# rzninvo/LGU-SLAM

Hardware: AMD Instinct MI355X
Metric: def-corr-sample Mpix·edges/s (48×64 fmap, r=3, L=4) (higher is better)
Workload: dtype f32; 1 GPU; BASELINE config 2: TartanAir-mono shape, 48x64 fmap, L=4, r=3, 20 edges per GPU, fused 4-level deformable sample; edges_per_gpu=20, variant=0, volumes=fmap products + avg_pool pyramid, pyramid_layout=4x8-tiled slices (CorrBlock's own storage; results bit-identical), out_format=planar, library=lgu_corr 0.8.0 gfx950

## Files before the change

### include/lgu_corr.h

```cpp
#ifndef LGU_CORR_H
#define LGU_CORR_H

#ifdef __cplusplus
extern "C" {
#endif

#define LGU_OK 0
#define LGU_E_BADARG 100001
#define LGU_E_UNSUPPORTED 100002

#define LGU_MAX_LEVELS 8
#define LGU_MAX_RADIUS 7

const char* lgu_version(void);
int lgu_debug_knobs_enabled(void);
const char* lgu_error_string(int code);


int lgu_defcorr_fwd_f32(const float* volume, const float* coords, float* offset, float* corr,
                        int E, int H1, int W1, int H2, int W2, int radius, void* stream);

int lgu_defcorr_bwd_f32(const float* volume, const float* coords, float* offset,
                        const float* corr_grad, float* volume_grad, float* offset_grad,
                        int E, int H1, int W1, int H2, int W2, int radius, void* stream);
// ... 59 lines not shown

int lgu_volume_pyramid_f32(const float* means, const float* covs, const float* volume, float* const* levels, int L,
                           int E, int H1, int W1, int H2, int W2, int radius, void* stream);

int lgu_volume_pyramid_tiled_f32(const float* means, const float* covs, const float* volume, float* const* levels,
                                 int L, int E, int H1, int W1, int H2, int W2, int radius, void* stream);

int lgu_volume_pyramid_h16(const float* means, const float* covs, const void* volume, float* const* levels, int L,
                           int E, int H1, int W1, int H2, int W2, int radius, int tiled, void* stream);

int lgu_volume_pyramid_det(const float* means, const float* covs, const void* det, int det_half, const void* volume,
                           int volume_half, float* const* levels, int L, int E, int H1, int W1, int H2, int W2, int radius,
                           int tiled, void* stream);

int lgu_volume_build_pyramid_f32(const float* fmap1, const float* fmap2, const float* means, const float* covs, const void* det,
                                 int det_half, float* const* levels, int L, int E, int C, int H, int W, int radius, void* stream);

int lgu_volume_build_pyramid_h16(const void* feats, void* workspace, const float* means, const float* covs, const void* det,
                                 int det_half, float* const* levels, int L, int E, int C, int H, int W, int radius, void* stream);

int lgu_volume_retile_f32(const float* src, float* dst, long long nslices, int H2, int W2, int to_tiled, void* stream);


int lgu_lowmem_defsample_fwd_f32(const float* fmap1, const float* fmap2, const float* coords,
                                 float* offset, float* corr,
                                 int B, int S, int H1, int W1, int H2, int W2, int C, int NO,
                                 int radius, void* stream);

int lgu_altcorr_fwd_f32(const float* fmap1, const float* fmap2, const float* coords, float* corr,
                        int B, int S, int H1, int W1, int H2, int W2, int C,
                        int radius, void* stream);

int lgu_altcorr_bwd_f32(const float* fmap1, const float* fmap2, const float* coords,
                        const float* corr_grad, float* fmap1_grad, float* fmap2_grad,
                        int B, int S, int H1, int W1, int H2, int W2, int C,
                        int radius, void* stream);

int lgu_lowmem_defsample_fwd_h16(const void* fmap1_half, const void* fmap2_half, const float* coords,
                                 float* offset, float* corr,
                                 int B, int S, int H1, int W1, int H2, int W2, int C, int NO,
                                 int radius, void* stream);
int lgu_altcorr_fwd_h16(const void* fmap1_half, const void* fmap2_half, const float* coords, float* corr,
                        int B, int S, int H1, int W1, int H2, int W2, int C,
                        int radius, void* stream);

int lgu_lowmem_pyramid_fwd_h16(const void* fmap1_half, const void* const* fmap2_half, const float* coords,
                               float* const* offsets, float* out,
                               int L, int lbase, int B, int S, int H1, int W1, const int* H2, const int* W2, int C, int NO,
                               int radius, const long long* ii, const long long* jj, void* stream);
int lgu_lowmem_pyramid_fwd_f32(const float* fmap1, const float* const* fmap2, const float* coords,
                               float* const* offsets, float* out,
                               int L, int lbase, int B, int S, int H1, int W1, const int* H2, const int* W2, int C, int NO,
                               int radius, const long long* ii, const long long* jj, void* stream);

int lgu_lowmem_pyramid_chunked_fwd_h16(const void* fmap1_half, const void* const* fmap2_half, const float* coords,
                                       float* const* offsets, float* out,
                                       int L, int lbase, int B, int S, int H1, int W1, const int* H2, const int* W2, int C, int NO,
                                       int radius, const long long* ii, const long long* jj, void* stream);
int lgu_lowmem_pyramid_chunked_fwd_f32(const float* fmap1, const float* const* fmap2, const float* coords,
                                       float* const* offsets, float* out,
                                       int L, int lbase, int B, int S, int H1, int W1, const int* H2, const int* W2, int C, int NO,
                                       int radius, const long long* ii, const long long* jj, void* stream);

int lgu_lowmem_pyramid_calls_fwd_h16(const void* fmap1_half, const void* const* fmap2_half, const float* coords,
                                     float* const* offsets, float* out,
                                     int L, int lbase, int B, int H1, int W1, const int* H2, const int* W2, int C, int NO,
                                     const int* off_row, int radius, const long long* ii, const long long* jj, int chunked,
                                     void* stream);

int lgu_ba_build_f32(const float* targets, const float* weights, const float* poses, const float* disps,
                     const float* intrinsics, const long long* ii, const long long* jj,
                     float* Hs, float* vs, float* Eii, float* Eij, float* Cii, float* wi, float* scratch,
                     int E, int ht, int wd, void* stream);
int lgu_ba_build_slices(int E);
int lgu_ba_accum_f32(const float* inp, const long long* ptrs, const long long* idxs, float* out, int nout, int D, void* stream);
int lgu_ba_depth_system_f32(const float* Cii, const float* wi, const long long* ptrs, const long long* idxs, const long long* kx,
                            const float* disps, const float* disps_sens, const float* eta, int eta_rows, float* Q, float* w,
                            int K, int HW, void* stream);
int lgu_ba_depth_update_f32(const float* Q, const float* w, const float* dw, const long long* ptrs, const long long* idxs,
                            const long long* kx, float* dz, float* disps, int K, int HW, void* stream);
int lgu_ba_scatter_sum_f64(const float* inp, const long long* ptrs, const long long* idxs, const long long* dst, double* out,
                           int m, int D, double sign, void* stream);
int lgu_ba_eet_f32(const float* E, const float* Q, const long long* idx, float* S, int nblocks, int D, void* stream);
int lgu_ba_ev_f32(const float* E, const float* Q, const float* w, const long long* kk, float* v, int n, int D, void* stream);
int lgu_ba_evt_f32(const float* E, const float* x, const long long* idx, float* dw, int n, int D, int P, void* stream);
int lgu_ba_solve_f64(const double* A, const double* b, float* x, int P, double lm, double ep, void* stream);
long long lgu_ba_solve_blocked_work_doubles(int P);
int lgu_ba_solve_blocked_f64(double* A, const double* b, float* x, double* work, int P, double lm, double ep, void* stream);
int lgu_ba_assemble_f64(const float* Hs, const long long* hptr, const long long* hidx, const float* S, const long long* sptr,
                        const long long* sidx, const float* vs, const long long* vptr, const long long* vidx, const float* sv,
                        const long long* svptr, const long long* svidx, double* Ad, double* b, int P, void* stream);
int lgu_ba_pose_retr_f32(float* poses, const float* dx, int t0, int t1, void* stream);
int lgu_ba_disp_retr_f32(float* disps, const float* dz, const long long* inds, int n, int HW, void* stream);

int lgu_frame_distance_f32(const float* poses, int np, const float* disps, int nd, int ht, int wd, const float* intrinsics,
                           const long long* ii, const long long* jj, int num, float beta, float* dist, void* stream);
int lgu_projmap_f32(const float* poses, int np, const float* disps, int nd, int ht, int wd, const float* intrinsics,
                    const long long* ii, const long long* jj, int num, float* coords, float* valid, void* stream);
int lgu_depth_filter_f32(const float* poses, int np, const float* disps, int nd, int ht, int wd, const float* intrinsics,
                         const long long* ix, const float* thresh, int num, float* counter, void* stream);
int lgu_iproj_f32(const float* poses, int np, const float* disps, int nd, int ht, int wd, const float* intrinsics,
                  float* points, void* stream);

#define LGU_REPROJ_JACOBIAN 1
#define LGU_REPROJ_DEPTH 2
int lgu_projective_transform_f32(const float* poses, const float* disps, const float* intrinsics, const long long* ii,
                                 const long long* jj, int B, int np, int nd, int ni, int ht, int wd, int num, int flags,
                                 float* coords, float* valid, float* Ji, float* Jj, float* Jz, void* stream);
int lgu_motion_features_f32(const float* poses, const float* disps, const float* intrinsics, const long long* ii,
                            const long long* jj, const float* target, int B, int np, int nd, int ni, int ht, int wd, int num,
                            float bound, float* coords1, float* motn, float* valid, void* stream);

#define LGU_UPS_MASK_F16 1
#define LGU_UPS_HALF_WEIGHTS 2
int lgu_scatter_mean_f32(const float* src, const long long* index, int outer, int n, long long inner, int M, float* out,
                         void* stream);
int lgu_scatter_mean_h16(const void* src, const long long* index, int outer, int n, long long inner, int M, void* out,
                         void* stream);
int lgu_cvx_upsample_f32(const float* data, const void* mask, int B, int ht, int wd, int flags, float* out, void* stream);
int lgu_upsample_disps_f32(const float* disps, int N, int ht, int wd, const long long* ix, int U, const void* mask,
                           int flags, float* disps_up, void* stream);

#define LGU_KANGRU_CTX_PIXELS 256
int lgu_kangru_context_f32(const float* net, const float* weight, const float* bias, int E, int HW, float* partial,
                           float* glo, void* stream);
int lgu_kangru_context_h16(const void* net, const void* weight, const void* bias, int E, int HW, float* partial, void* glo,
                           void* stream);
int lgu_kan_heads_f32(const float* glo, const float* grid, const float* wpack, int E, float* out, void* stream);
int lgu_kan_heads_h16(const void* glo, const float* grid, const void* wpack, int E, void* out, void* stream);
int lgu_kangru_gates_f32(const float* cz, const float* cr, const float* kz, const float* kr, const float* net, int E,
                         int HW, float* z, float* net_inp, void* stream);
int lgu_kangru_gates_h16(const void* cz, const void* cr, const void* kz, const void* kr, const void* net, int E, int HW,
                         void* z, void* net_inp, void* stream);
int lgu_kangru_blend_f32(const float* cq, const float* kq, const float* z, const float* net, int E, int HW, float* out,
                         void* stream);
int lgu_kangru_blend_h16(const void* cq, const void* kq, const void* z, const void* net, int E, int HW, void* out,
                         void* stream);

#define LGU_PROXIMITY_SMALL_MAX 4096
long long lgu_proximity_prefix_len(int t, int t0, int rad, int stereo);
long long lgu_proximity_capacity(int t, int t0, int t1, int rad, int stereo, long long max_factors);
long long lgu_proximity_work_bytes(int t, int t0, int t1);
int lgu_proximity_select_small(const float* dist, const long long* known_ii, const long long* known_jj, int num_known, int t,
                               int t0, int t1, int rad, int nms, double thresh, long long max_factors, int stereo,
                               long long* e_ii, long long* e_jj, long long capacity, int* count, void* stream);
int lgu_proximity_keys(const float* dist, const long long* known_ii, const long long* known_jj, int num_known, int t, int t0,
                       int t1, int rad, int nms, double thresh, int stereo, long long* keys, void* work, void* stream);
int lgu_proximity_select_sorted(const long long* sorted_keys, void* work, int t, int t0, int t1, int rad, int nms,
                                long long max_factors, int stereo, long long* e_ii, long long* e_jj, long long capacity,
                                int* count, void* stream);

#define LGU_LIE_SO3 0
#define LGU_LIE_SE3 1
int lgu_lie_inv_f32(int group, const float* G, int n, float* out, void* stream);
int lgu_lie_mul_f32(int group, const float* G, const float* H, int n, float* out, void* stream);
int lgu_lie_retr_f32(int group, const float* G, const float* a, int n, float* out, void* stream);
int lgu_lie_exp_f32(int group, const float* a, int n, float* out, void* stream);
int lgu_lie_log_f32(int group, const float* G, int n, float* out, void* stream);
int lgu_lie_matrix_f32(int group, const float* G, int n, float* out, void* stream);
int lgu_lie_act_f32(int group, const float* G, long long ng, const float* p, int width, long long rows, long long g_div,
                    float* out, void* stream);
int lgu_lie_adj_f32(int group, const float* G, long long ng, const float* a, int transpose, long long rows,
                    long long g_div, float* out, void* stream);

int lgu_instnorm_relu_f32(const float* a, const float* b, float* out, long planes, long hw, float eps, int mode,
                          void* stream);
// ... 98 lines not shown
```

### lgu-slam_amd/_lib.py

```python
import ctypes
import os

from . import _build

_c_float_p = ctypes.POINTER(ctypes.c_float)
_vp = ctypes.c_void_p
_int = ctypes.c_int


class FlowConv7Args(ctypes.Structure):
    _fields_ = [("x", _vp), ("wpack", _vp), ("bias", _vp), ("out", _vp), ("N", _int), ("H", _int), ("W", _int)]


class Conv3Args(ctypes.Structure):
    _fields_ = [("x", _vp), ("wpack", _vp), ("bias", _vp), ("out", _vp), ("N", _int), ("H", _int), ("W", _int),
                ("Cout", _int), ("flags", _int)]


class HeadArgs(ctypes.Structure):
    _fields_ = [("x", _vp), ("wpack", _vp), ("bias", _vp), ("out", _vp), ("N", _int), ("H", _int), ("W", _int),
                ("Cout", _int), ("flags", _int)]


class Conv3FanoutArgs(ctypes.Structure):
    _fields_ = [("x", _vp), ("wpack", _vp * 3), ("bias", _vp * 3), ("out", _vp * 3), ("N", _int), ("H", _int), ("W", _int),
                ("G", _int), ("flags", _int)]


class HeadPairArgs(ctypes.Structure):
    _fields_ = [("x", _vp * 2), ("wpack", _vp * 2), ("bias", _vp * 2), ("out", _vp * 2), ("coords", _vp), ("N", _int), ("H", _int),
                ("W", _int), ("flags", _int)]


class UpmaskArgs(ctypes.Structure):
    _fields_ = [("x", _vp), ("wpack", _vp), ("bias", _vp), ("out", _vp), ("N", _int), ("H", _int), ("W", _int), ("flags", _int)]


class UpmaskUpsArgs(ctypes.Structure):
    _fields_ = [("x", _vp), ("wpack", _vp), ("bias", _vp), ("disps", _vp), ("ix", _vp), ("disps_up", _vp), ("U", _int),
                ("N", _int), ("ht", _int), ("wd", _int), ("flags", _int)]


class Conv1Args(ctypes.Structure):
    _fields_ = [("x", _vp), ("wpack", _vp), ("bias", _vp), ("out", _vp), ("N", _int), ("Cin", _int), ("H", _int), ("W", _int),
                ("flags", _int)]


class GruConvArgs(ctypes.Structure):
    _fields_ = [("seg", _vp * 4), ("wpack", _vp), ("bias", _vp), ("k0", _vp), ("k1", _vp), ("net", _vp), ("z", _vp),
                ("out0", _vp), ("out1", _vp), ("seg_ch", _int * 4), ("nseg", _int), ("N", _int), ("H", _int), ("W", _int),
                ("Cout", _int), ("mode", _int), ("flags", _int)]


SIGNATURES = {
    "lgu_defcorr_fwd_f32": [_vp, _vp, _vp, _vp] + [_int] * 6 + [_vp],
    "lgu_defcorr_bwd_f32": [_vp] * 6 + [_int] * 6 + [_vp],
    "lgu_corridx_fwd_f32": [_vp, _vp, _vp] + [_int] * 6 + [_vp],
    "lgu_corridx_bwd_f32": [_vp] * 4 + [_int] * 6 + [_vp],
    "lgu_gaussmask_fwd_f32": [_vp] * 4 + [_int] * 6 + [_vp],
    "lgu_gaussmask_bwd_f32": [_vp] * 6 + [_int] * 6 + [_vp],
    "lgu_defcorr_pyramid_fwd_f32": [ctypes.POINTER(_vp), _vp, ctypes.POINTER(_vp), _vp, _int, _int, _int, _int,
                                    ctypes.POINTER(_int), ctypes.POINTER(_int), _int, _int, _vp],
    "lgu_defcorr_pyramid_slots_fwd_f32": [ctypes.POINTER(_vp), _vp, _vp, ctypes.POINTER(_vp), _vp, _int, _int, _int, _int,
                                          ctypes.POINTER(_int), ctypes.POINTER(_int), _int, _int, _vp],
    "lgu_volume_pyramid_f32": [_vp, _vp, _vp, ctypes.POINTER(_vp), _int, _int, _int, _int, _int, _int, _int, _vp],
    "lgu_volume_pyramid_tiled_f32": [_vp, _vp, _vp, ctypes.POINTER(_vp), _int, _int, _int, _int, _int, _int, _int, _vp],
    "lgu_volume_pyramid_h16": [_vp, _vp, _vp, ctypes.POINTER(_vp), _int, _int, _int, _int, _int, _int, _int, _int, _vp],
    "lgu_volume_pyramid_det": [_vp, _vp, _vp, _int, _vp, _int, ctypes.POINTER(_vp)] + [_int] * 8 + [_vp],
    "lgu_volume_build_pyramid_f32": [_vp] * 5 + [_int, ctypes.POINTER(_vp)] + [_int] * 6 + [_vp],
    "lgu_volume_build_pyramid_h16": [_vp] * 5 + [_int, ctypes.POINTER(_vp)] + [_int] * 6 + [_vp],
    "lgu_gaussian_params": [_vp] * 5 + [_int] * 4 + [ctypes.c_float, _vp],
    "lgu_probe_mask_scale_f32": [_vp, _vp, _int, _int, _int, _int, _vp],
    "lgu_offset_conv_frames_h16": [_vp] * 7 + [_int] * 5 + [_vp],
    "lgu_offset_heads_mark": [_vp, _vp, _int, _vp, _int, _vp, _vp, _vp],
    "lgu_offset_conv_worklist_h16": [_vp] * 4 + [_int] + [_vp] * 5 + [_int] * 4 + [_vp],
    "lgu_offset_heads_combine_f32": [_vp] * 5 + [_int] * 2 + [_vp, _vp],
    "lgu_offsets_finalize": [_vp] * 5 + [_int] * 7 + [ctypes.c_float, _vp],
    "lgu_offsets_finalize_masked": [_vp] * 3 + [_int] + [_vp] * 3 + [_int] * 7 + [ctypes.c_float, _vp],
    "lgu_volume_retile_f32": [_vp, _vp, ctypes.c_longlong, _int, _int, _int, _vp],
    "lgu_lowmem_defsample_fwd_f32": [_vp] * 5 + [_int] * 9 + [_vp],
    "lgu_altcorr_fwd_f32": [_vp] * 4 + [_int] * 8 + [_vp],
    "lgu_lowmem_defsample_fwd_h16": [_vp] * 5 + [_int] * 9 + [_vp],
    "lgu_altcorr_fwd_h16": [_vp] * 4 + [_int] * 8 + [_vp],
    "lgu_lowmem_pyramid_fwd_h16": [_vp, ctypes.POINTER(_vp), _vp, ctypes.POINTER(_vp), _vp, _int, _int, _int, _int, _int, _int,
                                   ctypes.POINTER(_int), ctypes.POINTER(_int), _int, _int, _int, _vp, _vp, _vp],
    "lgu_lowmem_pyramid_chunked_fwd_h16": [_vp, ctypes.POINTER(_vp), _vp, ctypes.POINTER(_vp), _vp, _int, _int, _int, _int, _int, _int,
                                   ctypes.POINTER(_int), ctypes.POINTER(_int), _int, _int, _int, _vp, _vp, _vp],
    "lgu_lowmem_pyramid_chunked_fwd_f32": [_vp, ctypes.POINTER(_vp), _vp, ctypes.POINTER(_vp), _vp, _int, _int, _int, _int, _int, _int,
                                   ctypes.POINTER(_int), ctypes.POINTER(_int), _int, _int, _int, _vp, _vp, _vp],
    "lgu_lowmem_pyramid_calls_fwd_h16": [_vp, ctypes.POINTER(_vp), _vp, ctypes.POINTER(_vp), _vp, _int, _int, _int, _int, _int,
                                         ctypes.POINTER(_int), ctypes.POINTER(_int), _int, _int, _vp, _int, _vp, _vp, _int, _vp],
    "lgu_lowmem_pyramid_fwd_f32": [_vp, ctypes.POINTER(_vp), _vp, ctypes.POINTER(_vp), _vp, _int, _int, _int, _int, _int, _int,
                                   ctypes.POINTER(_int), ctypes.POINTER(_int), _int, _int, _int, _vp, _vp, _vp],
    "lgu_ba_build_f32": [_vp] * 14 + [_int] * 3 + [_vp],
    "lgu_ba_build_slices": [_int],
    "lgu_ba_accum_f32": [_vp] * 4 + [_int] * 2 + [_vp],
    "lgu_ba_depth_system_f32": [_vp] * 8 + [_int] + [_vp] * 2 + [_int] * 2 + [_vp],
    "lgu_ba_depth_update_f32": [_vp] * 8 + [_int] * 2 + [_vp],
    "lgu_ba_scatter_sum_f64": [_vp] * 5 + [_int] * 2 + [ctypes.c_double, _vp],
    "lgu_ba_eet_f32": [_vp] * 4 + [_int] * 2 + [_vp],
    "lgu_ba_ev_f32": [_vp] * 5 + [_int] * 2 + [_vp],
    "lgu_ba_evt_f32": [_vp] * 4 + [_int] * 3 + [_vp],
    "lgu_ba_solve_f64": [_vp, _vp, _vp, _int, ctypes.c_double, ctypes.c_double, _vp],
    "lgu_ba_solve_blocked_f64": [_vp, _vp, _vp, _vp, _int, ctypes.c_double, ctypes.c_double, _vp],
    "lgu_ba_pose_retr_f32": [_vp] * 2 + [_int] * 2 + [_vp],
    "lgu_ba_assemble_f64": [_vp] * 14 + [_int, _vp],
    "lgu_ba_disp_retr_f32": [_vp] * 3 + [_int] * 2 + [_vp],
    "lgu_altcorr_bwd_f32": [_vp] * 6 + [_int] * 8 + [_vp],
    "lgu_defcorr_pyramid_enc_fwd_f32": [ctypes.POINTER(_vp), _vp, _vp, ctypes.POINTER(_vp), _vp, _vp, _vp, _int, _int, _int,
                                        _int, ctypes.POINTER(_int), ctypes.POINTER(_int), _int, _int, _int, _vp],
    "lgu_frame_distance_f32": [_vp, _int, _vp, _int, _int, _int, _vp, _vp, _vp, _int, ctypes.c_float, _vp, _vp],
    "lgu_projmap_f32": [_vp, _int, _vp, _int, _int, _int, _vp, _vp, _vp, _int, _vp, _vp, _vp],
    "lgu_depth_filter_f32": [_vp, _int, _vp, _int, _int, _int, _vp, _vp, _vp, _int, _vp, _vp],
    "lgu_iproj_f32": [_vp, _int, _vp, _int, _int, _int, _vp, _vp, _vp],
    "lgu_projective_transform_f32": [_vp] * 5 + [_int] * 8 + [_vp] * 6,
    "lgu_motion_features_f32": [_vp] * 6 + [_int] * 7 + [ctypes.c_float] + [_vp] * 4,
    "lgu_scatter_mean_f32": [_vp, _vp, _int, _int, ctypes.c_longlong, _int, _vp, _vp],
    "lgu_scatter_mean_h16": [_vp, _vp, _int, _int, ctypes.c_longlong, _int, _vp, _vp],
    "lgu_cvx_upsample_f32": [_vp, _vp] + [_int] * 4 + [_vp, _vp],
    "lgu_upsample_disps_f32": [_vp, _int, _int, _int, _vp, _int, _vp, _int, _vp, _vp],
    "lgu_kangru_context_f32": [_vp] * 3 + [_int] * 2 + [_vp] * 3,
    "lgu_kangru_context_h16": [_vp] * 3 + [_int] * 2 + [_vp] * 3,
    "lgu_kan_heads_f32": [_vp] * 3 + [_int] + [_vp] * 2,
    "lgu_kan_heads_h16": [_vp] * 3 + [_int] + [_vp] * 2,
    "lgu_kangru_gates_f32": [_vp] * 5 + [_int] * 2 + [_vp] * 3,
    "lgu_kangru_gates_h16": [_vp] * 5 + [_int] * 2 + [_vp] * 3,
    "lgu_kangru_blend_f32": [_vp] * 4 + [_int] * 2 + [_vp] * 2,
    "lgu_kangru_blend_h16": [_vp] * 4 + [_int] * 2 + [_vp] * 2,
    "lgu_proximity_select_small": [_vp] * 3 + [_int] * 6 + [ctypes.c_double, ctypes.c_longlong, _int, _vp, _vp,
                                                            ctypes.c_longlong, _vp, _vp],
    "lgu_proximity_keys": [_vp] * 3 + [_int] * 6 + [ctypes.c_double, _int, _vp, _vp, _vp],
    "lgu_proximity_select_sorted": [_vp] * 2 + [_int] * 5 + [ctypes.c_longlong, _int, _vp, _vp, ctypes.c_longlong, _vp, _vp],
    "lgu_lie_inv_f32": [_int, _vp, _int, _vp, _vp],
    "lgu_lie_mul_f32": [_int, _vp, _vp, _int, _vp, _vp],
    "lgu_lie_retr_f32": [_int, _vp, _vp, _int, _vp, _vp],
    "lgu_lie_exp_f32": [_int, _vp, _int, _vp, _vp],
    "lgu_lie_log_f32": [_int, _vp, _int, _vp, _vp],
    "lgu_lie_matrix_f32": [_int, _vp, _int, _vp, _vp],
    "lgu_lie_act_f32": [_int, _vp, ctypes.c_longlong, _vp, _int, ctypes.c_longlong, ctypes.c_longlong, _vp, _vp],
    "lgu_lie_adj_f32": [_int, _vp, ctypes.c_longlong, _vp, _int, ctypes.c_longlong, ctypes.c_longlong, _vp, _vp],
    "lgu_instnorm_relu_f32": [_vp] * 3 + [ctypes.c_long] * 2 + [ctypes.c_float, _int, _vp],
    "lgu_instnorm_relu_h16": [_vp] * 3 + [ctypes.c_long] * 2 + [ctypes.c_float, _int, _vp],
    "lgu_instnorm_resident_limit": [_int],
    "lgu_image_normalize_u8": [_vp, _vp, ctypes.c_long, ctypes.c_long, _c_float_p, _c_float_p, _vp],
    "lgu_flow_conv7_relu_h16": [FlowConv7Args, _vp],
    "lgu_conv3x3_c128_h16": [Conv3Args, _vp],
    "lgu_head3x3_c128_h16": [HeadArgs, _vp],
    "lgu_conv3x3_fanout_c128_h16": [Conv3FanoutArgs, _vp],
    "lgu_head3x3_pair_c128_h16": [HeadPairArgs, _vp],
    "lgu_gruconv3x3_c448_h16": [GruConvArgs, _vp],
    "lgu_upmask1x1_c128_h16": [UpmaskArgs, _vp],
    "lgu_upmask_upsample_f32": [UpmaskUpsArgs, _vp],
    "lgu_conv1x1_o128_h16": [Conv1Args, _vp],
    "lgu_ba_solve_blocked_work_doubles": [_int],
    "lgu_offsets_finalize_scratch_bytes": [_int],
    "lgu_proximity_prefix_len": [_int] * 4,
    "lgu_proximity_capacity": [_int] * 5 + [ctypes.c_longlong],
    "lgu_proximity_work_bytes": [_int] * 3,
    "lgu_version": [],
    "lgu_error_string": [_int],
    "lgu_debug_knobs_enabled": [],
}
RESTYPES = {name: ctypes.c_longlong for name in (
    "lgu_ba_solve_blocked_work_doubles", "lgu_offsets_finalize_scratch_bytes", "lgu_proximity_prefix_len", "lgu_proximity_capacity",
    "lgu_proximity_work_bytes")}
RESTYPES.update(lgu_instnorm_resident_limit=ctypes.c_long, lgu_version=ctypes.c_char_p, lgu_error_string=ctypes.c_char_p)

_lib = None


class LguLibraryError(RuntimeError):
    pass


class UnsupportedShape(RuntimeError):
    """The kernels do not serve this shape / argument pattern (LGU_E_UNSUPPORTED)."""


LGU_E_BADARG, LGU_E_UNSUPPORTED = 100001, 100002


def so_path():
    return os.environ.get("LGU_LIB_PATH") or _build.SO_PATH
# ... 36 lines not shown
```

### lgu-slam_amd/ba.py

```python
import os

import numpy as np
import torch

from . import _lib
from ._host import CurrentDevice, check_operands
from ._host import ptr as _ptr, stream as _stream

_ALPHA = 0.05


def _segments(ix, jx):
    ix = np.asarray(ix, dtype=np.int64)
    jx = np.asarray(jx, dtype=np.int64)
    order = np.argsort(ix, kind="stable")
    sx = ix[order]
    lo = np.searchsorted(sx, jx, side="left")
    hi = np.searchsorted(sx, jx, side="right")
    cnt = hi - lo
    ptrs = np.concatenate([[0], np.cumsum(cnt)])
    cols = np.concatenate([order[a:b] for a, b in zip(lo, hi)]) if len(jx) and cnt.sum() else np.zeros(0, np.int64)
    return ptrs, cols


class _Accum:

    def __init__(self, lib, ix, jx, dev):
        ptrs, cols = _segments(ix, jx)
        self.lib, self.n = lib, len(jx)
        self.ptrs = torch.from_numpy(np.ascontiguousarray(ptrs, dtype=np.int64)).to(dev)
        self.cols = torch.from_numpy(np.ascontiguousarray(cols if len(cols) else [0], dtype=np.int64)).to(dev)

    def __call__(self, data, st, out=None):
        if out is None:
            out = torch.empty((self.n, data.shape[1]), dtype=torch.float32, device=data.device)
        if self.n:
            _lib.check(self.lib.lgu_ba_accum_f32(_ptr(data), _ptr(self.ptrs), _ptr(self.cols), _ptr(out), self.n, data.shape[1], st),
                       "ba accum")
        return out


class _ScatterSum:

    def __init__(self, lib, dest, dev):
        dest = np.asarray(dest, dtype=np.int64)
        rows = np.nonzero(dest >= 0)[0]
        order = rows[np.argsort(dest[rows], kind="stable")]
        keys, counts = np.unique(dest[order], return_counts=True)
        ptrs = np.concatenate([[0], np.cumsum(counts)]).astype(np.int64)
        self.lib, self.m = lib, len(keys)
        self.ptrs = torch.from_numpy(ptrs).to(dev)
        self.idxs = torch.from_numpy(np.ascontiguousarray(order if len(order) else [0], dtype=np.int64)).to(dev)
        self.dst = torch.from_numpy(np.ascontiguousarray(keys if len(keys) else [0], dtype=np.int64)).to(dev)

    def __call__(self, inp, out, sign, st):
        if self.m:
            D = inp.shape[1]
            _lib.check(self.lib.lgu_ba_scatter_sum_f64(_ptr(inp), _ptr(self.ptrs), _ptr(self.idxs), _ptr(self.dst), _ptr(out), self.m, D,
                                                       float(sign), st), "ba assembly")


def _solve(A, b, lm, ep):
    L = A.clone()
    dg = torch.diagonal(L)
    dg += ep + lm * dg
    chol, info = torch.linalg.cholesky_ex(L)
    if int(info) != 0:
        return torch.zeros_like(b)
    return torch.cholesky_solve(b[:, None], chol)[:, 0]


def _csr(dest, ndst, dev):
    dest = np.asarray(dest, dtype=np.int64)
    rows = np.nonzero((dest >= 0) & (dest < ndst))[0]
    order = rows[np.argsort(dest[rows], kind="stable")]
    ptr = np.concatenate([[0], np.cumsum(np.bincount(dest[order], minlength=ndst))]).astype(np.int64)
    idx = np.ascontiguousarray(order if len(order) else [0], dtype=np.int64)
    return torch.from_numpy(ptr).to(dev), torch.from_numpy(idx).to(dev)


class _Plan:

    def __init__(self, lib, ii_h, jj_h, t0, t1, motion_only, dev):
        P = t1 - t0
        ts_h = np.arange(t0, t1, dtype=np.int64)
        ii_exp_h, jj_exp_h = np.concatenate([ts_h, ii_h]), np.concatenate([ts_h, jj_h])
        kx_h, kk_h = np.unique(ii_exp_h, return_inverse=True)
        kk_h = kk_h.astype(np.int64)
        self.kx = torch.from_numpy(kx_h).to(dev)
        self.kk = torch.from_numpy(kk_h).to(dev)
        self.K = int(kx_h.shape[0])
        bi_h = np.concatenate([ii_h, ii_h, jj_h, jj_h]) - t0
        bj_h = np.concatenate([ii_h, jj_h, ii_h, jj_h]) - t0
        self.csr_H = _csr(np.where((bi_h >= 0) & (bj_h >= 0) & (bi_h < P) & (bj_h < P), bi_h * P + bj_h, -1), P * P, dev)
        self.csr_v = _csr(np.concatenate([ii_h, jj_h]) - t0, P, dev)
        self.csr_S = self.csr_sv = None
        if motion_only:
            return
        ent = np.nonzero((jj_exp_h >= t0) & (jj_exp_h < t1))[0]
        ent = ent[np.argsort(kk_h[ent], kind="stable")]
        _, starts, sizes = np.unique(kk_h[ent], return_index=True, return_counts=True)
        a_l, c_l, k_l = [], [], []
        for s0, m_ in zip(starts, sizes):
            g = ent[s0:s0 + m_]
            ua, uc = np.triu_indices(m_)
            a_l.append(g[ua]); c_l.append(g[uc])
            k_l.append(np.full(len(ua), kk_h[g[0]], np.int64))
        self.have_pairs = len(a_l) > 0
        if self.have_pairs:
            a_n, c_n, k_n = np.concatenate(a_l), np.concatenate(c_l), np.concatenate(k_l)
        else:
            a_n = c_n = k_n = np.zeros(1, np.int64)
        self.trip_t = torch.from_numpy(np.ascontiguousarray(np.stack([a_n, c_n, k_n], 1))).to(dev)
        if self.have_pairs:
            npair = len(a_n)
            d_ac = (jj_exp_h[a_n] - t0) * P + (jj_exp_h[c_n] - t0)
            d_ca = np.where(a_n != c_n, (jj_exp_h[c_n] - t0) * P + (jj_exp_h[a_n] - t0), -1)
            ptr, idx = _csr(np.concatenate([d_ac, d_ca]), P * P, dev)
            self.csr_S = (ptr, torch.where(idx < npair, idx, npair - 1 - idx))
        else:
            self.csr_S = None
        self.csr_sv = _csr(jj_exp_h - t0, P, dev)
        self.jpose = torch.from_numpy(jj_exp_h - t0).to(dev).contiguous()
        self.acc_ii_kx = _Accum(lib, ii_h, kx_h, dev)
        self.acc_ii_ts = _Accum(lib, ii_h, ts_h, dev)
        self.acc_exp_kx = _Accum(lib, ii_exp_h, kx_h, dev)


_PLANS = {}
_PLANS_MAX = 8


def _plan_for(lib, ii, jj, t0, t1, motion_only, dev):
    ii_h, jj_h = ii.cpu().numpy().astype(np.int64), jj.cpu().numpy().astype(np.int64)
    key = (ii_h.tobytes(), jj_h.tobytes(), int(t0), int(t1), bool(motion_only), str(dev))
    plan = _PLANS.pop(key, None)
    if plan is None:
        plan = _Plan(lib, ii_h, jj_h, int(t0), int(t1), bool(motion_only), dev)
        while len(_PLANS) >= _PLANS_MAX:
            _PLANS.pop(next(iter(_PLANS)))
    _PLANS[key] = plan
    return plan


def _run(pl, lib, poses, disps, intrinsics, disps_sens, targets, weights, eta_v, ii, jj, t0, t1, iterations, lm, ep,
         motion_only, hooks=None):
    dev = poses.device
    E = ii.shape[0]
    ht, wd = disps.shape[1:]
    HW = ht * wd
    P = t1 - t0
    f32, f64 = torch.float32, torch.float64
    st = _stream(poses)
    kx, kk = pl.kx, pl.kk
    if not motion_only:
        have_pairs, trip_t, jpose = pl.have_pairs, pl.trip_t, pl.jpose
        acc_ii_kx, acc_ii_ts, acc_exp_kx = pl.acc_ii_kx, pl.acc_ii_ts, pl.acc_exp_kx
        K = pl.K
        Q = torch.empty((K, HW), dtype=f32, device=dev)
        w = torch.empty((K, HW), dtype=f32, device=dev)
    reduce_system, after_depth = hooks if hooks is not None else (None, None)
    Hs = torch.empty((4, max(E, 1), 6, 6), dtype=f32, device=dev)
    vs = torch.empty((2, max(E, 1), 6), dtype=f32, device=dev)
    Eii = torch.empty((max(E, 1), 6, HW), dtype=f32, device=dev)[:E]
    Eall = torch.empty((P + E, 6, HW), dtype=f32, device=dev)
    Eij = Eall[P:]
    scratch = torch.empty((max(E, 1) * lib.lgu_ba_build_slices(E) * 90,), dtype=f32, device=dev)
    Cii = torch.empty((max(E, 1), HW), dtype=f32, device=dev)[:E]
    wi = torch.empty((max(E, 1), HW), dtype=f32, device=dev)[:E]
    dx = torch.zeros((P, 6), dtype=f32, device=dev)
    dz = None
    for _ in range(iterations):
        if E:
          _lib.check(lib.lgu_ba_build_f32(_ptr(targets), _ptr(weights), _ptr(poses), _ptr(disps), _ptr(intrinsics), _ptr(ii),
                                          _ptr(jj), _ptr(Hs), _ptr(vs), _ptr(Eii), _ptr(Eij), _ptr(Cii), _ptr(wi), _ptr(scratch), E, ht, wd,
                                          st),
                     "ba build")
        S = sv = None
        if not motion_only:
            _lib.check(lib.lgu_ba_depth_system_f32(_ptr(Cii), _ptr(wi), _ptr(acc_ii_kx.ptrs), _ptr(acc_ii_kx.cols), _ptr(kx), _ptr(disps),
                                                   _ptr(disps_sens), _ptr(eta_v), eta_v.shape[0], _ptr(Q), _ptr(w), K, HW, st),
                       "ba depth system")
            acc_ii_ts(Eii.view(E, 6 * HW), st, out=Eall[:P].view(P, 6 * HW))
            nE = P + E
            if have_pairs:
                S = torch.empty((trip_t.shape[0], 6, 6), dtype=f32, device=dev)
                _lib.check(lib.lgu_ba_eet_f32(_ptr(Eall), _ptr(Q), _ptr(trip_t), _ptr(S), trip_t.shape[0], HW, st), "ba EEt")
            sv = torch.empty((nE, 6), dtype=f32, device=dev)
            _lib.check(lib.lgu_ba_ev_f32(_ptr(Eall), _ptr(Q), _ptr(w), _ptr(kk), _ptr(sv), nE, HW, st), "ba Ev")
        Ad = torch.empty((6 * P, 6 * P), dtype=f64, device=dev)
        b = torch.empty((P, 6), dtype=f64, device=dev)
        cS, cs = pl.csr_S if S is not None else None, pl.csr_sv if sv is not None else None
        _lib.check(lib.lgu_ba_assemble_f64(_ptr(Hs), _ptr(pl.csr_H[0]), _ptr(pl.csr_H[1]),
                                           _ptr(S) if S is not None else None, _ptr(cS[0]) if cS else None, _ptr(cS[1]) if cS else None,
                                           _ptr(vs), _ptr(pl.csr_v[0]), _ptr(pl.csr_v[1]),
                                           _ptr(sv) if sv is not None else None, _ptr(cs[0]) if cs else None, _ptr(cs[1]) if cs else None,
                                           _ptr(Ad), _ptr(b), P, st), "ba assembly")
        if reduce_system is not None:
            reduce_system(Ad, b)
        dx = torch.empty((P, 6), dtype=f32, device=dev)
        rc = lib.lgu_ba_solve_f64(_ptr(Ad), _ptr(b), _ptr(dx), P, float(lm), float(ep), st)
        if rc == _lib.LGU_E_UNSUPPORTED:
            if os.environ.get("LGU_BA_LIBRARY_SOLVE", "0") != "0":
                dx = _solve(Ad, b.view(-1), lm, ep).view(P, 6).to(f32).contiguous()
            else:
                work = torch.empty(int(lib.lgu_ba_solve_blocked_work_doubles(P)), dtype=f64, device=dev)
                _lib.check(lib.lgu_ba_solve_blocked_f64(_ptr(Ad), _ptr(b), _ptr(dx), _ptr(work), P, float(lm), float(ep), st),
                           "ba blocked solve")
        else:
            _lib.check(rc, "ba solve")
        if not motion_only:
            dw = torch.empty((nE, HW), dtype=f32, device=dev)
            _lib.check(lib.lgu_ba_evt_f32(_ptr(Eall), _ptr(dx), _ptr(jpose), _ptr(dw), nE, HW, P, st), "ba EvT")
            dz = torch.empty((K, HW), dtype=f32, device=dev)
            _lib.check(lib.lgu_ba_depth_update_f32(_ptr(Q), _ptr(w), _ptr(dw), _ptr(acc_exp_kx.ptrs), _ptr(acc_exp_kx.cols), _ptr(kx),
                                                   _ptr(dz), _ptr(disps), K, HW, st), "ba depth update")
            if after_depth is not None:
                after_depth(disps)
        _lib.check(lib.lgu_ba_pose_retr_f32(_ptr(poses), _ptr(dx), t0, t1, st), "ba pose retraction")
    return [dx, dz]


def ba(poses, disps, intrinsics, disps_sens, targets, weights, eta, ii, jj, t0, t1, iterations, lm, ep, motion_only, _hooks=None):
    named = [(poses, "poses"), (disps, "disps"), (intrinsics, "intrinsics"), (disps_sens, "disps_sens")]
    if ii.numel():
        named += [(targets, "targets"), (weights, "weights")]
    check_operands(named)
    check_operands([(ii, "ii")], torch.int64)
    check_operands([(jj, "jj")], torch.int64)
    lib = _lib.load()
    dev = poses.device
    HW = disps.shape[1] * disps.shape[2]
    with CurrentDevice(dev):
        pl = _plan_for(lib, ii, jj, t0, t1, motion_only, dev)
        eta_v = None
        if not motion_only:
            if callable(eta):
                eta = eta(pl.kx)
            eta_v = eta.reshape(-1, HW).to(torch.float32).contiguous()
            if eta_v.shape[0] not in (1, pl.K):
                raise RuntimeError("ba: eta must have one row per depth frame (%d) or one row, got %d" % (pl.K, eta_v.shape[0]))
        return _run(pl, lib, poses, disps, intrinsics, disps_sens, targets, weights, eta_v, ii, jj, t0, t1, iterations, lm, ep,
                    motion_only, _hooks)
```

### lgu-slam_amd/csrc/ba.hip

```cpp
#include "lgu_common.hpp"
#include "se3.hpp"

namespace lgu {

constexpr float BA_MIN_DEPTH = 0.25f;
constexpr int BA_THREADS = 256;

__device__ __forceinline__ void adj_se3(const float* t, const float* q, const float* X, float* Y) {
  const float qinv[4] = {-q[0], -q[1], -q[2], q[3]};
  act_so3(qinv, X, Y);
  act_so3(qinv, X + 3, Y + 3);
  const float u[3] = {t[2] * X[1] - t[1] * X[2], t[0] * X[2] - t[2] * X[0], t[1] * X[0] - t[0] * X[1]};
  float v[3];
  act_so3(qinv, u, v);
  Y[3] += v[0]; Y[4] += v[1]; Y[5] += v[2];
}

template <int N>
__device__ __forceinline__ float block_sums(const float (&v)[N], float* red ) {
  static_assert(N <= BA_THREADS, "one result per thread");
  const int w = threadIdx.x >> 6;
  __syncthreads();
#pragma unroll
  for (int i = 0; i < N; i++) {
// ... 188 lines not shown
    disps[f * D + k] += z;
  }
}

__global__ __launch_bounds__(BA_THREADS) void ba_scatter_sum_kernel(const float* __restrict__ inp, const long long* __restrict__ ptrs,
                                                                    const long long* __restrict__ idxs, const long long* __restrict__ dst,
                                                                    double* __restrict__ out, int m, int D, double sign) {
  const int t = blockIdx.x * BA_THREADS + threadIdx.x;
  if (t >= m * D) return;
  const int j = t / D, k = t - j * D;
  double acc = 0.0;
  for (long long i = ptrs[j]; i < ptrs[j + 1]; i++) acc += (double)inp[(size_t)idxs[i] * D + k];
  out[(size_t)dst[j] * D + k] += sign * acc;
}

__global__ __launch_bounds__(BA_THREADS) void ba_assemble_kernel(const float* __restrict__ Hs, const long long* __restrict__ hptr,
                                                                 const long long* __restrict__ hidx, const float* __restrict__ S,
                                                                 const long long* __restrict__ sptr, const long long* __restrict__ sidx,
                                                                 const float* __restrict__ vs, const long long* __restrict__ vptr,
                                                                 const long long* __restrict__ vidx, const float* __restrict__ sv,
                                                                 const long long* __restrict__ svptr, const long long* __restrict__ svidx,
                                                                 double* __restrict__ Ad, double* __restrict__ b, int P) {
  const long long t = (long long)blockIdx.x * BA_THREADS + threadIdx.x;
  const long long nA = (long long)P * P * 36;
  if (t < nA) {
    const int d = (int)(t / 36), k = (int)(t - (long long)d * 36);
    double a = 0.0;
    for (long long i = hptr[d]; i < hptr[d + 1]; i++) a += (double)Hs[(size_t)hidx[i] * 36 + k];
    double out = 0.0;
    if (hptr[d + 1] > hptr[d]) out += 1.0 * a;
    if (S) {
      double c = 0.0, ct = 0.0;
      bool anyd = false, anyt = false;
      const int kt = (k % 6) * 6 + k / 6;
      for (long long i = sptr[d]; i < sptr[d + 1]; i++) {
        const long long e = sidx[i];
        if (e >= 0) { c += (double)S[(size_t)e * 36 + k]; anyd = true; }
        else { ct += (double)S[(size_t)(-e - 1) * 36 + kt]; anyt = true; }
      }
      if (anyd) out += -1.0 * c;
      if (anyt) out += -1.0 * ct;
    }
    const int bi = d / P, bj = d - bi * P, r = k / 6, cidx = k - r * 6;
    Ad[((size_t)bi * 6 + r) * (6 * P) + bj * 6 + cidx] = out;
  } else if (t < nA + (long long)P * 6) {
    const int u = (int)(t - nA), d = u / 6, k = u - d * 6;
    double a = 0.0;
    for (long long i = vptr[d]; i < vptr[d + 1]; i++) a += (double)vs[(size_t)vidx[i] * 6 + k];
    double out = 0.0;
    if (vptr[d + 1] > vptr[d]) out += 1.0 * a;
    if (sv) {
      double c = 0.0;
      for (long long i = svptr[d]; i < svptr[d + 1]; i++) c += (double)sv[(size_t)svidx[i] * 6 + k];
      if (svptr[d + 1] > svptr[d]) out += -1.0 * c;
    }
    b[u] = out;
  }
}

__global__ __launch_bounds__(BA_THREADS) void ba_eet_kernel(const float* __restrict__ Em, const float* __restrict__ Q,
                                                            const long long* __restrict__ idx, float* __restrict__ S, int D) {
  __shared__ float red[4 * 36];
  const int ix = (int)idx[blockIdx.x * 3 + 0], jx = (int)idx[blockIdx.x * 3 + 1], kx = (int)idx[blockIdx.x * 3 + 2];
  float dS[36];
#pragma unroll
  for (int i = 0; i < 36; i++) dS[i] = 0.f;
  for (int k = threadIdx.x; k < D; k += BA_THREADS) {
    const float q = Q[(size_t)kx * D + k];
    float ei[6], ej[6];
#pragma unroll
    for (int n = 0; n < 6; n++) {
      ei[n] = Em[((size_t)ix * 6 + n) * D + k] * q;
      ej[n] = Em[((size_t)jx * 6 + n) * D + k];
    }
#pragma unroll
    for (int n = 0; n < 6; n++)
#pragma unroll
      for (int m = 0; m < 6; m++) dS[n * 6 + m] += ei[n] * ej[m];
  }
  const float ss = block_sums(dS, red);
  if (threadIdx.x < 36) S[(size_t)blockIdx.x * 36 + threadIdx.x] = ss;
}

__global__ __launch_bounds__(BA_THREADS) void ba_ev_kernel(const float* __restrict__ Em, const float* __restrict__ Q,
                                                           const float* __restrict__ w, const long long* __restrict__ kk,
                                                           float* __restrict__ v, int D) {
  __shared__ float red[4 * 6];
  const int kx = (int)kk[blockIdx.x];
  float b[6] = {0.f, 0.f, 0.f, 0.f, 0.f, 0.f};
  for (int k = threadIdx.x; k < D; k += BA_THREADS) {
    const float qw = Q[(size_t)kx * D + k] * w[(size_t)kx * D + k];
#pragma unroll
    for (int n = 0; n < 6; n++) b[n] += qw * Em[((size_t)blockIdx.x * 6 + n) * D + k];
  }
  const float sb = block_sums(b, red);
  if (threadIdx.x < 6) v[(size_t)blockIdx.x * 6 + threadIdx.x] = sb;
}

__global__ __launch_bounds__(BA_THREADS) void ba_evt_kernel(const float* __restrict__ Em, const float* __restrict__ x,
                                                            const long long* __restrict__ idx, float* __restrict__ dw, int D,
                                                            int P) {
  const int ix = (int)idx[blockIdx.x];
  const bool skip = ix <= 0 || ix >= P;
  float xr[6] = {0.f, 0.f, 0.f, 0.f, 0.f, 0.f};
  if (!skip)
#pragma unroll
    for (int n = 0; n < 6; n++) xr[n] = x[ix * 6 + n];
  for (int k = threadIdx.x; k < D; k += BA_THREADS) {
    float s = 0.f;
    if (!skip)
#pragma unroll
      for (int n = 0; n < 6; n++) s += Em[((size_t)blockIdx.x * 6 + n) * D + k] * xr[n];
    dw[(size_t)blockIdx.x * D + k] = s;
  }
}

__device__ __forceinline__ void exp_so3(const float* phi, float* q) {
  const float theta_sq = phi[0] * phi[0] + phi[1] * phi[1] + phi[2] * phi[2];
  const float theta_p4 = theta_sq * theta_sq, theta = sqrtf(theta_sq);
  float imag, real;
  if (theta_sq < 1e-8f) {
    imag = 0.5f - (1.0f / 48.0f) * theta_sq + (1.0f / 3840.0f) * theta_p4;
    real = 1.0f - (1.0f / 8.0f) * theta_sq + (1.0f / 384.0f) * theta_p4;
  } else {
    imag = sinf(0.5f * theta) / theta;
    real = cosf(0.5f * theta);
  }
  q[0] = imag * phi[0]; q[1] = imag * phi[1]; q[2] = imag * phi[2]; q[3] = real;
}
__global__ void ba_pose_retr_kernel(float* poses, const float* __restrict__ dx, int t0, int t1) {
  for (int k = t0 + blockIdx.x * blockDim.x + threadIdx.x; k < t1; k += gridDim.x * blockDim.x) {
    float xi[6], t[3], q[4], dt[3], dq[4], t1v[3], q1[4];
#pragma unroll
    for (int n = 0; n < 6; n++) xi[n] = dx[(k - t0) * 6 + n];
#pragma unroll
    for (int n = 0; n < 3; n++) t[n] = poses[k * 7 + n];
#pragma unroll
    for (int n = 0; n < 4; n++) q[n] = poses[k * 7 + 3 + n];
    exp_so3(xi + 3, dq);
    float tau[3] = {xi[0], xi[1], xi[2]}, tmp[3];
    const float* phi = xi + 3;
    const float theta_sq = phi[0] * phi[0] + phi[1] * phi[1] + phi[2] * phi[2], theta = sqrtf(theta_sq);
    dt[0] = tau[0]; dt[1] = tau[1]; dt[2] = tau[2];
    if (theta > 1e-4f) {
      const float a = (1 - cosf(theta)) / theta_sq;
      cross3(phi, tau, tmp); tau[0] = tmp[0]; tau[1] = tmp[1]; tau[2] = tmp[2];
      dt[0] += a * tau[0]; dt[1] += a * tau[1]; dt[2] += a * tau[2];
      const float b = (theta - sinf(theta)) / (theta * theta_sq);
      cross3(phi, tau, tmp); tau[0] = tmp[0]; tau[1] = tmp[1]; tau[2] = tmp[2];
      dt[0] += b * tau[0]; dt[1] += b * tau[1]; dt[2] += b * tau[2];
    }
    q1[0] = dq[3] * q[0] + dq[0] * q[3] + dq[1] * q[2] - dq[2] * q[1];
    q1[1] = dq[3] * q[1] + dq[1] * q[3] + dq[2] * q[0] - dq[0] * q[2];
    q1[2] = dq[3] * q[2] + dq[2] * q[3] + dq[0] * q[1] - dq[1] * q[0];
    q1[3] = dq[3] * q[3] - dq[0] * q[0] - dq[1] * q[1] - dq[2] * q[2];
    act_so3(dq, t, t1v);
#pragma unroll
    for (int n = 0; n < 3; n++) poses[k * 7 + n] = t1v[n] + dt[n];
#pragma unroll
    for (int n = 0; n < 4; n++) poses[k * 7 + 3 + n] = q1[n];
  }
}

__global__ __launch_bounds__(BA_THREADS) void ba_disp_retr_kernel(float* disps, const float* __restrict__ dz,
                                                                  const long long* __restrict__ inds, int HW) {
  const size_t f = (size_t)inds[blockIdx.x];
// ... 163 lines not shown
  return launch_status();
}

int lgu_ba_build_f32(const float* targets, const float* weights, const float* poses, const float* disps,
                     const float* intrinsics, const long long* ii, const long long* jj, float* Hs, float* vs, float* Eii,
                     float* Eij, float* Cii, float* wi, float* scratch, int E, int ht, int wd, void* stream) {
  using namespace lgu;
  if (!targets || !weights || !poses || !disps || !intrinsics || !ii || !jj || !Hs || !vs || !Eii || !Eij || !Cii || !wi || !scratch)
    return LGU_E_BADARG;
  if (E < 0 || ht < 1 || wd < 1) return LGU_E_BADARG;
  if (E == 0) return LGU_OK;
  hipStream_t st = reinterpret_cast<hipStream_t>(stream);
  const int slices = lgu_ba_build_slices(E);
  hipLaunchKernelGGL(ba_build_kernel, dim3(E, slices), dim3(BA_THREADS), 0, st, targets, weights, poses, disps, intrinsics, ii, jj,
                     scratch, Eii, Eij, Cii, wi, E, ht * wd, wd, slices);
  hipLaunchKernelGGL(ba_build_finalize_kernel, dim3((E * 90 + BA_THREADS - 1) / BA_THREADS), dim3(BA_THREADS), 0, st, scratch, Hs, vs, E,
                     slices);
  return launch_status();
}

int lgu_ba_accum_f32(const float* inp, const long long* ptrs, const long long* idxs, float* out, int nout, int D, void* stream) {
  using namespace lgu;
  if (!inp || !ptrs || !out || nout < 0 || D < 1) return LGU_E_BADARG;
  if (nout == 0) return LGU_OK;
  hipLaunchKernelGGL(ba_accum_kernel, dim3(nout, (D + BA_THREADS * 4 - 1) / (BA_THREADS * 4)), dim3(BA_THREADS), 0,
                     reinterpret_cast<hipStream_t>(stream), inp, ptrs, idxs, out, D);
  return launch_status();
}

int lgu_ba_depth_system_f32(const float* Cii, const float* wi, const long long* ptrs, const long long* idxs, const long long* kx,
                            const float* disps, const float* disps_sens, const float* eta, int eta_rows, float* Q, float* w, int K,
                            int HW, void* stream) {
  using namespace lgu;
  if (!Cii || !wi || !ptrs || !idxs || !kx || !disps || !disps_sens || !eta || !Q || !w || K < 0 || HW < 1) return LGU_E_BADARG;
  if (eta_rows != 1 && eta_rows != K) return LGU_E_BADARG;
  if (K == 0) return LGU_OK;
  hipLaunchKernelGGL(ba_depth_system_kernel, dim3(K, (HW + BA_THREADS * 4 - 1) / (BA_THREADS * 4)), dim3(BA_THREADS), 0,
                     reinterpret_cast<hipStream_t>(stream), Cii, wi, ptrs, idxs, kx, disps, disps_sens, eta, eta_rows, 0.05f, Q, w, HW);
  return launch_status();
}

int lgu_ba_depth_update_f32(const float* Q, const float* w, const float* dw, const long long* ptrs, const long long* idxs,
                            const long long* kx, float* dz, float* disps, int K, int HW, void* stream) {
  using namespace lgu;
  if (!Q || !w || !dw || !ptrs || !idxs || !kx || !dz || !disps || K < 0 || HW < 1) return LGU_E_BADARG;
  if (K == 0) return LGU_OK;
  hipLaunchKernelGGL(ba_depth_update_kernel, dim3(K, (HW + BA_THREADS * 4 - 1) / (BA_THREADS * 4)), dim3(BA_THREADS), 0,
                     reinterpret_cast<hipStream_t>(stream), Q, w, dw, ptrs, idxs, kx, dz, disps, HW);
  return launch_status();
}

int lgu_ba_scatter_sum_f64(const float* inp, const long long* ptrs, const long long* idxs, const long long* dst, double* out, int m,
                           int D, double sign, void* stream) {
  using namespace lgu;
  if (!inp || !ptrs || !idxs || !dst || !out || m < 0 || D < 1) return LGU_E_BADARG;
  if (m == 0) return LGU_OK;
  const unsigned grid = (unsigned)(((size_t)m * D + BA_THREADS - 1) / BA_THREADS);
  hipLaunchKernelGGL(ba_scatter_sum_kernel, dim3(grid), dim3(BA_THREADS), 0, reinterpret_cast<hipStream_t>(stream), inp, ptrs, idxs,
                     dst, out, m, D, sign);
  return launch_status();
}

int lgu_ba_assemble_f64(const float* Hs, const long long* hptr, const long long* hidx, const float* S, const long long* sptr,
                        const long long* sidx, const float* vs, const long long* vptr, const long long* vidx, const float* sv,
                        const long long* svptr, const long long* svidx, double* Ad, double* b, int P, void* stream) {
  using namespace lgu;
  if (!Hs || !hptr || !hidx || !vs || !vptr || !vidx || !Ad || !b || P < 1) return LGU_E_BADARG;
  if ((S && (!sptr || !sidx)) || (sv && (!svptr || !svidx))) return LGU_E_BADARG;
  const long long n = (long long)P * P * 36 + (long long)P * 6;
  hipLaunchKernelGGL(ba_assemble_kernel, dim3((unsigned)((n + BA_THREADS - 1) / BA_THREADS)), dim3(BA_THREADS), 0,
                     reinterpret_cast<hipStream_t>(stream), Hs, hptr, hidx, S, sptr, sidx, vs, vptr, vidx, sv, svptr, svidx, Ad, b, P);
  return launch_status();
}

int lgu_ba_eet_f32(const float* Em, const float* Q, const long long* idx, float* S, int nblocks, int D, void* stream) {
  using namespace lgu;
  if (!Em || !Q || !S || nblocks < 0 || D < 1) return LGU_E_BADARG;
  if (nblocks == 0) return LGU_OK;
  if (!idx) return LGU_E_BADARG;
  hipLaunchKernelGGL(ba_eet_kernel, dim3(nblocks), dim3(BA_THREADS), 0, reinterpret_cast<hipStream_t>(stream), Em, Q, idx, S, D);
  return launch_status();
}

int lgu_ba_ev_f32(const float* Em, const float* Q, const float* w, const long long* kk, float* v, int n, int D, void* stream) {
  using namespace lgu;
  if (!Em || !Q || !w || !kk || !v || n < 0 || D < 1) return LGU_E_BADARG;
  if (n == 0) return LGU_OK;
  hipLaunchKernelGGL(ba_ev_kernel, dim3(n), dim3(BA_THREADS), 0, reinterpret_cast<hipStream_t>(stream), Em, Q, w, kk, v, D);
  return launch_status();
}

int lgu_ba_evt_f32(const float* Em, const float* x, const long long* idx, float* dw, int n, int D, int P, void* stream) {
  using namespace lgu;
  if (!Em || !x || !idx || !dw || n < 0 || D < 1 || P < 1) return LGU_E_BADARG;
  if (n == 0) return LGU_OK;
  hipLaunchKernelGGL(ba_evt_kernel, dim3(n), dim3(BA_THREADS), 0, reinterpret_cast<hipStream_t>(stream), Em, x, idx, dw, D, P);
  return launch_status();
}

int lgu_ba_pose_retr_f32(float* poses, const float* dx, int t0, int t1, void* stream) {
  using namespace lgu;
  if (!poses || !dx || t0 < 0 || t1 < t0) return LGU_E_BADARG;
  if (t1 == t0) return LGU_OK;
  hipLaunchKernelGGL(ba_pose_retr_kernel, dim3((t1 - t0 + 63) / 64), dim3(64), 0, reinterpret_cast<hipStream_t>(stream), poses, dx,
                     t0, t1);
  return launch_status();
}

int lgu_ba_disp_retr_f32(float* disps, const float* dz, const long long* inds, int n, int HW, void* stream) {
  using namespace lgu;
  if (!disps || !dz || !inds || n < 0 || HW < 1) return LGU_E_BADARG;
  if (n == 0) return LGU_OK;
  hipLaunchKernelGGL(ba_disp_retr_kernel, dim3(n), dim3(BA_THREADS), 0, reinterpret_cast<hipStream_t>(stream), disps, dz, inds, HW);
  return launch_status();
}

}
```

Before: 1263 Mpix·edges/s.

## Group bundle-adjustment EEt triplets into runs sharing the i-side row

Adds a run-based EEt kernel that groups consecutive triplets sharing the same (i, k) indices so each block loads the Q-weighted Ei row once and reuses it across up to G j-rows. It also swizzles block IDs across eight groups. The run table is built on the host during planning. With the default BA_EET_G of 1, every run has length one, so the path behaves like the old per-triplet kernel plus the swizzle and extra indirection. The benchmarked metric is deformable correlation sampling, which this bundle-adjustment code does not touch.

```diff
diff --git a/include/lgu_corr.h b/include/lgu_corr.h
--- a/include/lgu_corr.h
+++ b/include/lgu_corr.h
@@ -165,6 +165,12 @@
 int lgu_ba_scatter_sum_f64(const float* inp, const long long* ptrs, const long long* idxs, const long long* dst, double* out,
                            int m, int D, double sign, void* stream);
 int lgu_ba_eet_f32(const float* E, const float* Q, const long long* idx, float* S, int nblocks, int D, void* stream);
+typedef struct {
+  const float* E; const float* Q; const long long* idx; const long long* runs; float* S;
+  int nitems, D;
+} lgu_ba_eet_runs_args;
+int lgu_ba_eet_runs_f32(lgu_ba_eet_runs_args args, void* stream);
+int lgu_ba_eet_runs_group(void);
 int lgu_ba_ev_f32(const float* E, const float* Q, const float* w, const long long* kk, float* v, int n, int D, void* stream);
 int lgu_ba_evt_f32(const float* E, const float* x, const long long* idx, float* dw, int n, int D, int P, void* stream);
 int lgu_ba_solve_f64(const double* A, const double* b, float* x, int P, double lm, double ep, void* stream);
diff --git a/lgu-slam_amd/_lib.py b/lgu-slam_amd/_lib.py
--- a/lgu-slam_amd/_lib.py
+++ b/lgu-slam_amd/_lib.py
@@ -50,6 +50,10 @@
     _fields_ = [("seg", _vp * 4), ("wpack", _vp), ("bias", _vp), ("k0", _vp), ("k1", _vp), ("net", _vp), ("z", _vp),
                 ("out0", _vp), ("out1", _vp), ("seg_ch", _int * 4), ("nseg", _int), ("N", _int), ("H", _int), ("W", _int),
                 ("Cout", _int), ("mode", _int), ("flags", _int)]
+
+
+class BaEetRunsArgs(ctypes.Structure):
+    _fields_ = [("E", _vp), ("Q", _vp), ("idx", _vp), ("runs", _vp), ("S", _vp), ("nitems", _int), ("D", _int)]
 
 
 SIGNATURES = {
@@ -99,6 +103,8 @@
     "lgu_ba_depth_update_f32": [_vp] * 8 + [_int] * 2 + [_vp],
     "lgu_ba_scatter_sum_f64": [_vp] * 5 + [_int] * 2 + [ctypes.c_double, _vp],
     "lgu_ba_eet_f32": [_vp] * 4 + [_int] * 2 + [_vp],
+    "lgu_ba_eet_runs_f32": [BaEetRunsArgs, _vp],
+    "lgu_ba_eet_runs_group": [],
     "lgu_ba_ev_f32": [_vp] * 5 + [_int] * 2 + [_vp],
     "lgu_ba_evt_f32": [_vp] * 4 + [_int] * 3 + [_vp],
     "lgu_ba_solve_f64": [_vp, _vp, _vp, _int, ctypes.c_double, ctypes.c_double, _vp],
diff --git a/lgu-slam_amd/ba.py b/lgu-slam_amd/ba.py
--- a/lgu-slam_amd/ba.py
+++ b/lgu-slam_amd/ba.py
@@ -77,6 +77,25 @@
     ptr = np.concatenate([[0], np.cumsum(np.bincount(dest[order], minlength=ndst))]).astype(np.int64)
     idx = np.ascontiguousarray(order if len(order) else [0], dtype=np.int64)
     return torch.from_numpy(ptr).to(dev), torch.from_numpy(idx).to(dev)
+
+
+def _eet_runs(a_n, k_n, group):
+    a_n, k_n = np.asarray(a_n, dtype=np.int64), np.asarray(k_n, dtype=np.int64)
+    n = len(a_n)
+    if n == 0:
+        return np.zeros((0, 3), np.int64)
+    first = np.flatnonzero(np.concatenate([[True], (a_n[1:] != a_n[:-1]) | (k_n[1:] != k_n[:-1])]))
+    length = np.diff(np.concatenate([first, [n]]))
+    pieces = (length + group - 1) // group
+    run = np.repeat(np.arange(len(first)), pieces)
+    piece = np.arange(len(run)) - np.repeat(np.cumsum(pieces) - pieces, pieces)
+    start = first[run] + piece * group
+    count = np.minimum(group, length[run] - piece * group)
+    return np.ascontiguousarray(np.stack([start, count, start], 1))
+
+
+def _use_eet_runs():
+    return not (_lib.debug_knobs_enabled() and os.environ.get("LGU_BA_EET_RUNS", "1") == "0")
 
 
 class _Plan:
@@ -112,7 +131,9 @@
         else:
             a_n = c_n = k_n = np.zeros(1, np.int64)
         self.trip_t = torch.from_numpy(np.ascontiguousarray(np.stack([a_n, c_n, k_n], 1))).to(dev)
+        self.runs_t = None
         if self.have_pairs:
+            self.runs_t = torch.from_numpy(_eet_runs(a_n, k_n, int(lib.lgu_ba_eet_runs_group()))).to(dev)
             npair = len(a_n)
             d_ac = (jj_exp_h[a_n] - t0) * P + (jj_exp_h[c_n] - t0)
             d_ca = np.where(a_n != c_n, (jj_exp_h[c_n] - t0) * P + (jj_exp_h[a_n] - t0), -1)
@@ -157,6 +178,7 @@
         have_pairs, trip_t, jpose = pl.have_pairs, pl.trip_t, pl.jpose
         acc_ii_kx, acc_ii_ts, acc_exp_kx = pl.acc_ii_kx, pl.acc_ii_ts, pl.acc_exp_kx
         K = pl.K
+        eet_runs = _use_eet_runs()
         Q = torch.empty((K, HW), dtype=f32, device=dev)
         w = torch.empty((K, HW), dtype=f32, device=dev)
     reduce_system, after_depth = hooks if hooks is not None else (None, None)
@@ -185,7 +207,11 @@
             nE = P + E
             if have_pairs:
                 S = torch.empty((trip_t.shape[0], 6, 6), dtype=f32, device=dev)
-                _lib.check(lib.lgu_ba_eet_f32(_ptr(Eall), _ptr(Q), _ptr(trip_t), _ptr(S), trip_t.shape[0], HW, st), "ba EEt")
+                if eet_runs:
+                    _lib.check(lib.lgu_ba_eet_runs_f32(_lib.BaEetRunsArgs(Eall.data_ptr(), Q.data_ptr(), trip_t.data_ptr(), pl.runs_t.data_ptr(),
+                                                                          S.data_ptr(), pl.runs_t.shape[0], HW), st), "ba EEt by runs")
+                else:
+                    _lib.check(lib.lgu_ba_eet_f32(_ptr(Eall), _ptr(Q), _ptr(trip_t), _ptr(S), trip_t.shape[0], HW, st), "ba EEt")
             sv = torch.empty((nE, 6), dtype=f32, device=dev)
             _lib.check(lib.lgu_ba_ev_f32(_ptr(Eall), _ptr(Q), _ptr(w), _ptr(kk), _ptr(sv), nE, HW, st), "ba Ev")
         Ad = torch.empty((6 * P, 6 * P), dtype=f64, device=dev)
diff --git a/lgu-slam_amd/csrc/ba.hip b/lgu-slam_amd/csrc/ba.hip
--- a/lgu-slam_amd/csrc/ba.hip
+++ b/lgu-slam_amd/csrc/ba.hip
@@ -294,6 +294,59 @@
   if (threadIdx.x < 36) S[(size_t)blockIdx.x * 36 + threadIdx.x] = ss;
 }
 
+#ifndef BA_EET_G
+#define BA_EET_G 1
+#endif
+template <int L>
+__device__ __forceinline__ void eet_run(const float* __restrict__ Em, const float* __restrict__ Q, const long long* __restrict__ idx,
+                                        float* __restrict__ S, int D, long long start, long long row, float* red) {
+  const int ix = (int)idx[start * 3 + 0], kx = (int)idx[start * 3 + 2];
+  int jx[L];
+  float dS[L][36];
+#pragma unroll
+  for (int c = 0; c < L; c++) {
+    jx[c] = (int)idx[(start + c) * 3 + 1];
+#pragma unroll
+    for (int i = 0; i < 36; i++) dS[c][i] = 0.f;
+  }
+  for (int k = threadIdx.x; k < D; k += BA_THREADS) {
+    const float q = Q[(size_t)kx * D + k];
+    float ei[6];
+#pragma unroll
+    for (int n = 0; n < 6; n++) ei[n] = Em[((size_t)ix * 6 + n) * D + k] * q;
+#pragma unroll
+    for (int c = 0; c < L; c++) {
+      float ej[6];
+#pragma unroll
+      for (int m = 0; m < 6; m++) ej[m] = Em[((size_t)jx[c] * 6 + m) * D + k];
+#pragma unroll
+      for (int n = 0; n < 6; n++)
+#pragma unroll
+        for (int m = 0; m < 6; m++) dS[c][n * 6 + m] += ei[n] * ej[m];
+    }
+  }
+#pragma unroll
+  for (int c = 0; c < L; c++) {
+    const float ss = block_sums(dS[c], red);
+    if (threadIdx.x < 36) S[(size_t)(row + c) * 36 + threadIdx.x] = ss;
+  }
+}
+
+__global__ __launch_bounds__(BA_THREADS) void ba_eet_runs_kernel(const float* __restrict__ Em, const float* __restrict__ Q,
+                                                                 const long long* __restrict__ idx, const long long* __restrict__ runs,
+                                                                 float* __restrict__ S, int D) {
+  __shared__ float red[4 * 36];
+  unsigned bid = blockIdx.x;
+  const unsigned n8 = gridDim.x & ~7u;
+  if (bid < n8) bid = (bid & 7u) * (n8 >> 3) + (bid >> 3);
+  const long long start = runs[(size_t)bid * 3 + 0], len = runs[(size_t)bid * 3 + 1], row = runs[(size_t)bid * 3 + 2];
+  static_assert(BA_EET_G >= 1 && BA_EET_G <= 4, "one instantiation per group length");
+  if (len == 1) eet_run<1>(Em, Q, idx, S, D, start, row, red);
+  else if (len == 2 && BA_EET_G >= 2) eet_run<2>(Em, Q, idx, S, D, start, row, red);
+  else if (len == 3 && BA_EET_G >= 3) eet_run<3>(Em, Q, idx, S, D, start, row, red);
+  else if (len == 4 && BA_EET_G >= 4) eet_run<4>(Em, Q, idx, S, D, start, row, red);
+}
+
 __global__ __launch_bounds__(BA_THREADS) void ba_ev_kernel(const float* __restrict__ Em, const float* __restrict__ Q,
                                                            const float* __restrict__ w, const long long* __restrict__ kk,
                                                            float* __restrict__ v, int D) {
@@ -623,6 +676,18 @@
   return launch_status();
 }
 
+int lgu_ba_eet_runs_group(void) { return BA_EET_G; }
+
+int lgu_ba_eet_runs_f32(lgu_ba_eet_runs_args a, void* stream) {
+  using namespace lgu;
+  if (!a.E || !a.Q || !a.S || a.nitems < 0 || a.D < 1) return LGU_E_BADARG;
+  if (a.nitems == 0) return LGU_OK;
+  if (!a.idx || !a.runs) return LGU_E_BADARG;
+  hipLaunchKernelGGL(ba_eet_runs_kernel, dim3(a.nitems), dim3(BA_THREADS), 0, reinterpret_cast<hipStream_t>(stream), a.E, a.Q, a.idx,
+                     a.runs, a.S, a.D);
+  return launch_status();
+}
+
 int lgu_ba_ev_f32(const float* Em, const float* Q, const float* w, const long long* kk, float* v, int n, int D, void* stream) {
   using namespace lgu;
   if (!Em || !Q || !w || !kk || !v || n < 0 || D < 1) return LGU_E_BADARG;
```

Measured after the change: 1261 Mpix·edges/s. Within noise of the previous version (-0.2%).
